# RichealYoung/BRIEF_PyTorch

Hardware: AMD Instinct MI355X
Metric: encode_voxels_per_sec (higher is better)
Workload: dtype f32; 1 GPU; SingleTask 512^3 synthetic uint16 volume, SIREN 4x256 (layers=5, features=256, w0=20), randompoint sample_size=100000, datal2, Adamax lr=1e-3; layers=5, features=256, sample_size=100000, params=198657

## Files before the change

__graft_entry__.py:

```python
import os
import subprocess
import sys

ROOT = os.path.dirname(os.path.abspath(__file__))
if ROOT not in sys.path:
    sys.path.insert(0, ROOT)


def build():
    from brief_pytorch_amd import _lib
    _lib.build(verbose=True)
    subprocess.check_call(["make", "-s", "-C", os.path.join(ROOT, "oracle")])
    import brief_pytorch_amd
    L = _lib.lib()
    for name in _lib.EXPORTS:
        assert hasattr(L, name), name
    print("build ok: libbrief_hip.so version", L.brief_version())


def smoke():
    import numpy as np
    import torch
    from brief_pytorch_amd import _lib
    from brief_pytorch_amd.networks import SIREN
    from brief_pytorch_amd.synthetic import make_volume
    from oracle import oracle as O

    assert torch.cuda.is_available(), "smoke() needs a GPU"
    _lib.lib()
    dims = (12, 16, 20)
    vol = make_volume(dims, seed=1)
    vn, side = O.normalize(vol)
    n = int(np.prod(dims))
    tv = torch.from_numpy(vn.reshape(-1, 1)).cuda()
    for layers, feats in ((5, 256), (4, 64), (3, 1100)):
        torch.manual_seed(0)
        m = SIREN(coords_channel=3, data_channel=1, features=feats, layers=layers, w0=20)
        d = O.make_desc(3, 1, layers, feats, 20.0)
        p = m.params.numpy().copy()
        m.to("cuda")
        loss, _ = m.train_step(n, tv, grid=(dims, -1.0, 1.0))
        lo, go, _, _ = O.loss_grad(d, p, O.grid_coords(dims), vn.reshape(-1, 1))
        g = m.grads.cpu().numpy()
        assert abs(loss.item() - lo) / lo < 1e-5, (loss.item(), lo)
# ... 12 lines not shown
```

brief_pytorch_amd/_lib.py:

```python
import ctypes as C
import os
import subprocess

_HERE = os.path.dirname(os.path.abspath(__file__))
LIB_PATH = os.environ.get("BRIEF_LIB", os.path.join(_HERE, "libbrief_hip.so"))
SRC = os.path.join(_HERE, "csrc", "brief_hip.hip")
_CSRC = os.path.join(_HERE, "csrc")
_DEPS = sorted(os.path.join(_CSRC, f) for f in (os.listdir(_CSRC) if os.path.isdir(_CSRC) else []) if f.endswith((".hip", ".inc", ".h"))) \
    + [os.path.join(os.path.dirname(_HERE), "include", "brief_hip.h")]
HIPCC = os.environ.get("HIPCC", "/opt/rocm/bin/hipcc")


class BriefError(RuntimeError):
    pass


class SirenDesc(C.Structure):
    _fields_ = [("cin", C.c_int32), ("cout", C.c_int32), ("layers", C.c_int32), ("features", C.c_int32),
                ("w0_first", C.c_float), ("w0_hidden", C.c_float), ("output_act", C.c_int32), ("precision", C.c_int32)]


class GridDesc(C.Structure):
    _fields_ = [("ndim", C.c_int32), ("reserved", C.c_int32), ("dims", C.c_int64 * 3), ("lo", C.c_float), ("hi", C.c_float)]

# ... 65 lines not shown

EXPORTS = ["brief_version", "brief_last_error", "brief_param_count", "brief_packed_count",
           "brief_train_workspace_bytes", "brief_siren_repack", "brief_siren_forward", "brief_forward_workspace_bytes", "brief_siren_forward_ws", "brief_siren_forward_box", "brief_siren_train_step", "brief_siren_fit_step",
           "brief_siren_fit", "brief_multi_fit",
           "brief_optim_step", "brief_sample_indices", "brief_sse_u16", "brief_profile_enable", "brief_profile_fused", "brief_deblock_edge", "brief_ssim_u16", "brief_ssim_partial_count",
           "brief_sincos_probe", "brief_cu_count",
           "brief_ffn_param_count", "brief_ffn_packed_count", "brief_ffn_train_workspace_bytes", "brief_ffn_repack", "brief_ffn_forward",
           "brief_ffn_forward_box", "brief_ffn_train_step", "brief_ffn_fit",
           "brief_nerf_param_count", "brief_nerf_packed_count", "brief_nerf_train_workspace_bytes", "brief_nerf_repack", "brief_nerf_forward",
           "brief_nerf_forward_box", "brief_nerf_train_step", "brief_nerf_fit",
           "brief_mfn_param_count", "brief_mfn_packed_count", "brief_mfn_train_workspace_bytes", "brief_mfn_repack", "brief_mfn_forward",
           "brief_mfn_forward_box", "brief_mfn_train_step", "brief_mfn_fit",
           "brief_taper_param_count", "brief_taper_packed_count", "brief_taper_train_workspace_bytes", "brief_taper_repack",
           "brief_taper_forward", "brief_taper_forward_box", "brief_taper_train_step", "brief_taper_fit",
           "brief_correct_chunk_elems", "brief_correct_count", "brief_correct_emit", "brief_correct_apply"]


def needs_build():
    if LIB_PATH != os.path.join(_HERE, "libbrief_hip.so"):
        return False
    if not os.path.exists(LIB_PATH):
        return True
    t = os.path.getmtime(LIB_PATH)
    return any(os.path.exists(d) and os.path.getmtime(d) > t for d in _DEPS)


DIAG_LIB_PATH = os.path.join(_HERE, "libbrief_hip_diag.so")


def build(force=False, verbose=False, diagnostics=False, defines=(), out=None):
    target = out or (DIAG_LIB_PATH if diagnostics else os.path.join(_HERE, "libbrief_hip.so"))
    if not force and not diagnostics and not defines and out is None and not needs_build():
        return LIB_PATH
    cmd = [HIPCC, "--offload-arch=gfx950", "-O3", "-std=c++17", "-ffp-contract=off", "-shared", "-fPIC", SRC, "-o", target]
    if diagnostics:
        cmd.append("-DBRIEF_DIAGNOSTICS")
    cmd += ["-D" + d for d in defines]
    if verbose:
        print(" ".join(cmd))
    subprocess.check_call(cmd)
    return target


_LIB = None


def lib():
    global _LIB
    if _LIB is not None:
        return _LIB
    import torch
    if not os.path.exists(LIB_PATH):
        raise BriefError("libbrief_hip.so is not built (run `python -c 'import __graft_entry__ as g; g.build()'`); "
                         "there is no CPU fallback for the fused SIREN path")
    L = C.CDLL(LIB_PATH)
    dp, gp, bp, vp = C.POINTER(SirenDesc), C.POINTER(GridDesc), C.POINTER(BatchDesc), C.c_void_p
    L.brief_version.restype = C.c_int
    if L.brief_version() != 130:
        raise BriefError("libbrief_hip.so is version %d, this binding needs 130 (brief_siren_forward_ws, widths to 4096): rebuild with __graft_entry__.build()" % L.brief_version())
    L.brief_last_error.restype = C.c_char_p
    L.brief_param_count.restype = C.c_int64
    L.brief_param_count.argtypes = [dp]
    L.brief_packed_count.restype = C.c_int64
    L.brief_packed_count.argtypes = [dp]
    L.brief_train_workspace_bytes.restype = C.c_int64
    L.brief_train_workspace_bytes.argtypes = [dp, C.c_int64]
# ... 89 lines not shown
```

brief_pytorch_amd/csrc/brief_device.inc:

```
typedef float f32x16 __attribute__((ext_vector_type(16)));
#define MFMA(a, b, c) __builtin_amdgcn_mfma_f32_32x32x2f32((a), (b), (c), 0, 0, 0)

#define ROWMAP(r, hi) (((r) & 3) + 8 * ((r) >> 2) + 4 * (hi))
template <int V> struct RoleC { static constexpr int value = V; };

template <int NT, bool INFER = false>
struct KCfg {
    static constexpr int WM = INFER ? brief_wm_infer(NT) : brief_wm(NT);
    static constexpr int WS = 4 / WM;
    static constexpr int MTW = (NT + WM - 1) / WM;
    static constexpr bool EXACT = (NT % WM) == 0;
    static constexpr int FP = 32 * NT;
    static constexpr int XS_FLOATS = WS * NT * 1024;
    static constexpr int TROWS = 32 * MTW;
    static constexpr int RS = (TROWS + 63) / 64;
    static constexpr int T_FLOATS = 4 * TROWS * 33;
    static constexpr int G_FLOATS = 4 * 256;
};

struct GridArgs {
    int ndim;
    int64_t dims[3];
    float lo, hi;
    float step[3];
// ... 12 lines not shown
    return dv == 1 ? nn : (uint32_t)__umul64hi(magic, (uint64_t)nn);
}

struct FusedArgs {
    brief_siren_desc d;
    const float *pk;
    const float *coords;
    const float *targets;
    const float *weights;
    const int64_t *idx;
    int64_t offset;
    int64_t n;
    uint64_t rng_pop, rng_seed, rng_step;
    GridArgs grid;
    int loss_kind;
    float thr, beta, inv_count;
    float *Z;
    float *D;
    int64_t npad;
    float *rec;
    int64_t n_begin, n_end;
    int rec_base;
    void *S16[5];
    float *slabs;
    float *yhat_out;
    void *out;
    int out_kind;
    float scale_min, den, span, vmin;
    int stagger_cus;
    int stagger;
    int pers_wgs;
    int64_t pers_tiles;
    int diag;
};
struct FusedBoxArgs : FusedArgs {
    BoxArgs box;
};
template <bool BOX> struct KArgsT { using type = FusedArgs; };
template <> struct KArgsT<true> { using type = FusedBoxArgs; };
typedef const __attribute__((address_space(4))) FusedBoxArgs *kargs_box;

__device__ __forceinline__ void lds_barrier()
{
    asm volatile("s_waitcnt lgkmcnt(0)" ::: "memory");
    __builtin_amdgcn_s_barrier();
    asm volatile("" ::: "memory");
}

__device__ __forceinline__ float lin_coord(const GridArgs &g, int a, int64_t i)
{
    const int64_t nn = g.dims[a];
    if (nn == 1) return g.lo;
    return i < nn / 2 ? __fmaf_rn(g.step[a], (float)i, g.lo) : __fmaf_rn(-g.step[a], (float)(nn - 1 - i), g.hi);
}

__device__ __forceinline__ float lin_coord32(const GridArgs &g, int a, uint32_t i)
{
    const uint32_t nn = (uint32_t)g.dims[a];
    if (nn == 1) return g.lo;
    return i < nn / 2 ? __fmaf_rn(g.step[a], (float)i, g.lo) : __fmaf_rn(-g.step[a], (float)(nn - 1 - i), g.hi);
}

__device__ __forceinline__ void grid_coords(const GridArgs &g, int cin, int64_t j, float &x0, float &x1, float &x2)
{
    if (cin == 3) {
        int64_t id, ih, iw;
        if (g.fast) {
// ... 135 lines not shown
                }
        }
        if (it + 1 < NIT) breg[it + 1] = Xs[(it + 1) * 64 + lane];
        __builtin_amdgcn_sched_barrier(0);
        const float4 b = breg[it];
#pragma unroll
        for (int t = 0; t < K::MTW; ++t) {
            if (K::EXACT || wm + K::WM * t < NT) {
                const float4 a = areg[it][t];
                acc[t] = MFMA(a.x, b.x, acc[t]);
                acc[t] = MFMA(a.y, b.y, acc[t]);
                acc[t] = MFMA(a.z, b.z, acc[t]);
                acc[t] = MFMA(a.w, b.w, acc[t]);
            }
        }
    }
}

template <int NT, bool INFER = false>
__device__ __forceinline__ void write_image(float4 *Xs, const f32x16 (&h)[(KCfg<NT, INFER>::MTW)], int wm, int lane)
{
    using K = KCfg<NT, INFER>;
#pragma unroll
    for (int t = 0; t < K::MTW; ++t) {
        const int mt = wm + K::WM * t;
        if (K::EXACT || mt < NT) {
#pragma unroll
            for (int q = 0; q < 4; ++q)
                Xs[(mt * 4 + q) * 64 + lane] = make_float4(h[t][4 * q], h[t][4 * q + 1], h[t][4 * q + 2], h[t][4 * q + 3]);
        }
    }
}

__device__ __forceinline__ void philox_round(uint32_t (&c)[4], uint32_t k0, uint32_t k1)
{
    const uint64_t p0 = (uint64_t)0xD2511F53u * c[0], p1 = (uint64_t)0xCD9E8D57u * c[2];
    const uint32_t n0 = (uint32_t)(p1 >> 32) ^ c[1] ^ k0, n1 = (uint32_t)p1;
    const uint32_t n2 = (uint32_t)(p0 >> 32) ^ c[3] ^ k1, n3 = (uint32_t)p0;
    c[0] = n0; c[1] = n1; c[2] = n2; c[3] = n3;
}

__device__ __forceinline__ int64_t philox_index(int64_t i, uint64_t pop, uint64_t seed, uint64_t step)
{
    uint32_t c[4] = {(uint32_t)i, (uint32_t)((uint64_t)i >> 32), (uint32_t)step, (uint32_t)(step >> 32)};
    uint32_t k0 = (uint32_t)seed, k1 = (uint32_t)(seed >> 32);
#pragma unroll
    for (int r = 0; r < 10; ++r) {
        philox_round(c, k0, k1);
        k0 += 0x9E3779B9u; k1 += 0xBB67AE85u;
    }
    const uint64_t r64 = ((uint64_t)c[0] << 32) | c[1];
    return (int64_t)__umul64hi(r64, pop);
}

#ifndef BRIEF_FUSED64
#ifndef BRIEF_LEAN_RM3
#define BRIEF_LEAN_RM3 1
#endif
#define BRIEF_FUSED64 0
#endif
#ifndef BRIEF_KERNARG_RELOAD
#define BRIEF_KERNARG_RELOAD 1
#endif
#ifndef BRIEF_TRAIN_WPE
#define BRIEF_TRAIN_WPE 2
#endif
// ... 6 lines not shown
```

brief_pytorch_amd/csrc/brief_fused.inc:

```
template <int NT, bool INFER = false>
struct FusedLds {
    using K = KCfg<NT, INFER>;
    static constexpr int R_FLOATS = K::XS_FLOATS > K::T_FLOATS ? K::XS_FLOATS : K::T_FLOATS;
    static constexpr int G_OFF = R_FLOATS;
    static constexpr int HW_OFF = G_OFF + K::G_FLOATS;
    static constexpr int TOTAL = HW_OFF + 4 * K::FP + 4;
};

#ifndef BRIEF_LEAN
#define BRIEF_LEAN 1
#endif
#ifndef BRIEF_LEAN7
#define BRIEF_LEAN7 0
#endif
constexpr bool fused_lean(int NT) { return BRIEF_LEAN && (NT == 8 || NT == BRIEF_LEAN7); }
constexpr int fused_train_wpe(int NT) { return NT > 8 ? 1 : (NT <= 4 || fused_lean(NT) ? (BRIEF_TRAIN_WPE > 3 ? BRIEF_TRAIN_WPE : 3) : BRIEF_TRAIN_WPE); }
template <int NT, bool TRAIN, bool BOX = false>
__global__ __launch_bounds__(256, TRAIN ? fused_train_wpe(NT) : (NT > 8 ? 2 : 3)) void k_fused(const typename KArgsT<BOX>::type a)
{
    static_assert(!(TRAIN && BOX), "the box mapping is an inference instantiation");
#ifdef BRIEF_STAMPS
    float st_acc[10] = {0.f, 0.f, 0.f, 0.f, 0.f, 0.f, 0.f, 0.f, 0.f, 0.f};
    long long st_last = clock64();
    const long long st_c0 = st_last, st_r0 = wall_clock64();
#endif
    using K = KCfg<NT, !TRAIN>;
    using LD = FusedLds<NT, !TRAIN>;
    extern __shared__ __attribute__((aligned(16))) float smem[];
    float4 *X = reinterpret_cast<float4 *>(smem);
    float *T = smem;
    float *G = smem + LD::G_OFF;
    float *HW = smem + LD::HW_OFF;

    const int lane = threadIdx.x & 63;
    const int wave = __builtin_amdgcn_readfirstlane(threadIdx.x >> 6);
    const int hi = lane >> 5, ln = lane & 31;
    const int wm = wave % K::WM, ws = wave / K::WM;
    const brief_siren_desc &d = a.d;
    const int L = d.layers, cin = d.cin, cout = d.cout;
    const int kit = (d.features + 7) >> 3;
    const int64_t npad = a.npad;
    const float *pk = a.pk;
    float4 *Xs = X + ws * (NT * 256);
    float *Tw = T + wave * (K::TROWS * 33);
    float *Gw = G + wave * 256;
    const float4 *W0p = reinterpret_cast<const float4 *>(pk + brief_pk_w0(d));
    const __amdgpu_buffer_rsrc_t rs_pk =
        __builtin_amdgcn_make_buffer_rsrc((void *)pk, 0, (int)(brief_pk_count(d) * 4), 0x00020000);
    const int stash_bytes = (a.diag & 1) ? 0 : (int)((int64_t)K::FP * npad * 4);
// ... 328 lines not shown
                if (K::EXACT || mt < NT) {
#pragma unroll
                    for (int r = 0; r < 16; ++r)
                        dl[t][r] = acc[t][r] * BRIEF_COS_REV(zr[t][r]);
                }
            }
        }
        STAMP(7)
        lds_barrier();
#pragma unroll
        for (int t = 0; t < K::MTW; ++t) {
#pragma unroll
            for (int r = 0; r < 16; ++r) Tw[(32 * t + ROWMAP(r, hi)) * 33 + ln] = dl[t][r];
        }
        lds_barrier();
#pragma unroll
        for (int rs = 0; rs < K::RS; ++rs) {
            float4 s0 = make_float4(0.f, 0.f, 0.f, 0.f);
            const int row = lane + 64 * rs;
            const float *trow = Tw + (row < K::TROWS ? row : 0) * 33;
#pragma unroll 4
            for (int s = 0; s < 32; ++s) {
                const float dv = trow[s];
                const float4 xv = *reinterpret_cast<const float4 *>(Gw + 128 + s * 4);
                s0.x = __fmaf_rn(dv, xv.x, s0.x); s0.y = __fmaf_rn(dv, xv.y, s0.y);
                s0.z = __fmaf_rn(dv, xv.z, s0.z); s0.w = __fmaf_rn(dv, xv.w, s0.w);
            }
            if (row < K::TROWS) { acc0[rs][0] += s0.x; acc0[rs][1] += s0.y; acc0[rs][2] += s0.z; acc0[rs][3] += s0.w; }
        }
        lds_barrier();
        STAMP(6)
    }
#undef FUSED_LOAD_BIAS
    if (TRAIN) {
        float *rec = a.rec + (((int64_t)blockIdx.x + a.rec_base) * 4 + wave) * BRIEF_REC_FLOATS;
#pragma unroll
        for (int rs = 0; rs < K::RS; ++rs) {
            const int row = lane + 64 * rs;
            if (row < 128) {
#pragma unroll
                for (int c = 0; c < 4; ++c) {
                    rec[row * 4 + c] = acc0[rs][c];
                    rec[BRIEF_REC_DWH + c * 128 + row] = accWh[rs][c];
                }
            }
        }
        for (int off = 32; off >= 1; off >>= 1) lsum += __shfl_xor(lsum, off);
        if (lane == 0) {
#pragma unroll
            for (int c = 0; c < 4; ++c) rec[BRIEF_REC_DBH + c] = accbh[c];
            rec[BRIEF_REC_LOSS] = lsum;
#ifdef BRIEF_STAMPS
            for (int i = 0; i < 10; ++i) rec[BRIEF_REC_STAMPS + i] = st_acc[i];
            rec[BRIEF_REC_STAMPS + 10] = (float)(clock64() - st_c0);
            rec[BRIEF_REC_STAMPS + 11] = (float)(wall_clock64() - st_r0);
            rec[BRIEF_REC_STAMPS + 12] = (float)(st_r0 & 0xFFFFFF);
            rec[BRIEF_REC_STAMPS + 13] = (float)(__builtin_amdgcn_s_getreg(20 | (0 << 6) | (3 << 11)) & 15);
            rec[BRIEF_REC_STAMPS + 14] = (float)(__builtin_amdgcn_s_getreg(4 | (0 << 6) | (15 << 11)) & 0xFFFF);
#endif
        }
    }
}
```

brief_pytorch_amd/csrc/brief_hip.hip:

```cpp
#include <hip/hip_runtime.h>
#include <hip/hip_ext.h>
#include <stdint.h>
#include <stdio.h>
#include <string.h>
#include <stdlib.h>
#include <mutex>
#include "brief_layout.h"
#include "brief_math.h"

#include "brief_device.inc"
#include "brief_fused.inc"
#include "brief_lean.inc"
#include "brief_wide.inc"
#include "brief_small.inc"
#include "brief_wgrad.inc"
#include "brief_x3.inc"
#include "brief_reduce.inc"
#include "brief_bf16.inc"
#include "brief_aux.inc"
#include "brief_ffn.inc"
#include "brief_nerf.inc"
#include "brief_mfn.inc"
#include "brief_taper.inc"
#include "brief_correct.inc"
// ... 117 lines not shown
static const bool g_wg_per_cu_set = env_str("BRIEF_WG_PER_CU") != nullptr;
static const int g_stagger = env_int("BRIEF_STAGGER", 0, 0, 64);
static const int g_diag = env_int("BRIEF_DIAG", 0, 0, 255);
static const int g_x3_decode = env_int("BRIEF_X3_DECODE", 1, 0, 1);
static const int g_wgrad_repeat = env_int("BRIEF_WGRAD_REPEAT", 1, 1, 8);
static const int g_reduce_sg_big = env_int("BRIEF_REDUCE_SG_BIG", 4, 1, 64);
static const int g_reduce_part = env_int("BRIEF_REDUCE_PART", 0, 0, 2);
static const int g_reduce_vec = env_int("BRIEF_REDUCE_VEC", 1, 0, 1);
static const int g_reduce_sg_small = env_int("BRIEF_REDUCE_SG", 0, 0, 64);
static int64_t fused_wg_samples(const brief_siren_desc &d, bool train)
{
    if (brief_use_wide(d)) return 32;
    if (d.precision == BRIEF_PREC_F32 && brief_use_lean(d, train)) return 32;
    if (!train && d.precision == BRIEF_PREC_F32) return 32 * (4 / brief_wm_infer(brief_nt(d)));
    return brief_wg_samples(brief_nt(d));
}
static int fused_grid(const brief_siren_desc &d, int64_t n, bool train)
{
    const int nt = brief_nt(d);
    const int64_t wgs_ = fused_wg_samples(d, train);
    const int64_t tiles = (n + wgs_ - 1) / wgs_;
    const int wpe = g_wg_per_cu_set ? g_wg_per_cu : (d.precision == BRIEF_PREC_BF16X3 && (train || g_x3_decode) ? 2  :
                    (BRIEF_FUSED64 && train && nt == 8 ? (BRIEF_FUSED64 == 1 ? 2 : 3)  : (train ? fused_train_wpe(nt) : (nt > 8 ? 2 : 3))));
    int64_t cap = (int64_t)kCUs * (train && nt > 8 ? 1 : wpe);
    if (brief_use_wide(d)) cap = kCUs;
    if (d.precision == BRIEF_PREC_F32 && brief_use_lean(d, train))
    {
        const int64_t by_lds = (160 * 1024) / (int64_t)(sizeof(float) * lean_lds(1, (nt + 3) / 4, nt).total);
        const int64_t by_regs = lean_wpe(1, (nt + 3) / 4);
        cap = (int64_t)kCUs * (by_lds < by_regs ? (by_lds > 0 ? by_lds : 1) : by_regs);
    }
    return (int)(tiles < cap ? (tiles > 0 ? tiles : 1) : cap);
}
struct FusedPlan { int grid, pers_wgs; int64_t pers_tiles; };
static const int g_tail_rounds = env_int("BRIEF_TAIL_ROUNDS", 0, 0, 64);
static FusedPlan fused_plan(const brief_siren_desc &d, int64_t n, bool train)
{
    const int nt = brief_nt(d);
    const int64_t wgs_ = fused_wg_samples(d, train);
    const int64_t tiles = (n + wgs_ - 1) / wgs_;
    const int cap = fused_grid(d, n, train);
    FusedPlan p;
    p.grid = cap; p.pers_wgs = cap; p.pers_tiles = tiles;
    if (!train || nt > 8 || tiles <= cap || brief_use_wide(d)) return p;
    if (g_tail_rounds == 0) return p;
    int64_t rounds = tiles / cap - g_tail_rounds;
    if (rounds < 0) rounds = 0;
    const int64_t max_wgs = (int64_t)kCUs * kRecWgsPerCu;
    while (tiles - rounds * cap + (rounds ? cap : 0) > max_wgs) ++rounds;
    if (rounds * cap >= tiles) return p;
    p.pers_wgs = rounds ? cap : 0;
    p.pers_tiles = rounds * cap;
    p.grid = p.pers_wgs + (int)(tiles - p.pers_tiles);
    return p;
}
#ifndef BRIEF_WGRAD_ROUNDS
#define BRIEF_WGRAD_ROUNDS 1
#endif
#ifndef BRIEF_TAIL_PLAN
#define BRIEF_TAIL_PLAN 1
#endif
#ifndef BRIEF_TAIL_LEAN
#define BRIEF_TAIL_LEAN 0
#endif
#ifndef BRIEF_TAIL_MODE_DEFAULT
#define BRIEF_TAIL_MODE_DEFAULT 2
#endif
#ifndef BRIEF_TAIL_R
#define BRIEF_TAIL_R 1.15
#define BRIEF_TAIL_R1 1.05
#endif
#ifndef BRIEF_TAIL_MIN_SPLITS
#define BRIEF_TAIL_MIN_SPLITS 6
#endif
#ifndef BRIEF_TAIL_MIN_ROUNDS
#define BRIEF_TAIL_MIN_ROUNDS 3
#endif
struct TailPlan { int mode ; bool on; int grid_body, grid_tail; int64_t tiles_body; int ns, n_norm; int64_t kfix_n, kfix_s; };
// ... 13 lines not shown
    const int64_t full = tiles / G * G, rem = tiles - full;
    if (full == 0 || rem == 0) return p;
    if (g_tail_mode == 2 && nt >= 9 && nt <= g_tail_ntmax && rem * 4 <= 3 * (int64_t)kCUs) {
        const int hidden = d.layers - 2, nq = wgrad_nq(nt), qt = (nt + nq - 1) / nq;
        const int64_t chunks = brief_npad_d(d, n) / 32, B = (int64_t)hidden * nq * nq;
        int ns = wgrad_split_rule(d, chunks, 1);
        if ((int64_t)ns * B > kCUs) ns = (int)(kCUs / B);
        const int per_xcd = kCUs / 8, tail_x = (int)((rem + 7) / 8);
        int n_norm = 0;
        if ((int64_t)ns * B <= kCUs)
            for (int c = ns - 1; c >= 1; --c) {
                const int a_ = (int)((c * B + 7) / 8), s_ = (int)(((ns - c) * B + 7) / 8);
                if (a_ + tail_x <= per_xcd && a_ + s_ <= per_xcd && (ns - c) * B >= rem) { n_norm = c; break; }
            }
        const int n_short = ns - n_norm;
        const double r = g_tail_r ? 0.01 * g_tail_r : (nt <= 16 ? BRIEF_TAIL_R : BRIEF_TAIL_R1);
        const double rho = r * 2.0 * hidden * nt * nt / (double)(qt * qt);
        const double k_norm = ((double)chunks + n_short * rho) / ns, k_short = k_norm - rho;
        if (n_norm > 0 && k_short >= 4.0 && rho < 0.8 * k_norm) {
            p.kfix_n = (int64_t)(k_norm * 65536.0); p.kfix_s = (int64_t)(k_short * 65536.0);
            const int64_t b_norm = ((int64_t)(ns - n_short) * p.kfix_n) >> 16;
            if (b_norm <= full && b_norm > 0) {
                p.mode = 2; p.on = true; p.grid_body = G; p.grid_tail = (int)rem; p.tiles_body = full; p.ns = ns; p.n_norm = ns - n_short;
                return p;
            }
        }
    }
    if (!(brief_use_wide(d) || (BRIEF_TAIL_LEAN && brief_use_lean(d, true) && nt >= 9))) return p;
    if (rem * 4 > 3 * (int64_t)G) return p;
    if (wgrad_split_rule(d, full, BRIEF_TAIL_MIN_ROUNDS) < BRIEF_TAIL_MIN_SPLITS) return p;
    p.mode = 1; p.on = true; p.grid_body = G; p.grid_tail = (int)rem; p.tiles_body = full;
    return p;
}
static int wgrad_split_rule(const brief_siren_desc &d, int64_t nchunks, int min_rounds)
{
    const int hidden = d.layers - 2;
    if (hidden <= 0) return 0;
    const int nq = wgrad_nq(brief_nt(d));
    const int64_t B = (int64_t)hidden * nq * nq;
    int64_t s = kWgradBlocks / B;
    if (s < 1) s = 1;
    if (min_rounds > 1) {
        double best = 1e30;
        for (int64_t c = 1; c <= 64; ++c) {
            const int64_t rounds = (c * B + kWgradBlocks - 1) / kWgradBlocks;
            if (rounds < min_rounds && c < 64) continue;
            const double cost = (double)rounds / (double)c + 0.0001 * (double)c;
            if (cost < best - 1e-9) { best = cost; s = c; }
        }
    } else if (brief_nt(d) > 32) {
        double best = 1e30;
        for (int64_t c = 1; c <= 16; ++c) {
            const double cost = (double)((c * B + kWgradBlocks - 1) / kWgradBlocks) / (double)c + 0.001 * (double)c;
            if (cost < best - 1e-9) { best = cost; s = c; }
        }
    } else if (nq >= 2 && BRIEF_WGRAD_ROUNDS) {
        const double base = 1.0 / (double)s + 0.0001 * (double)s;
        double best = base;
        const int64_t cmax = 4 * s > 16 ? 4 * s : 16;
        for (int64_t c = s + 1; c <= cmax && c <= 64; ++c) {
            const double cost = (double)((c * B + kWgradBlocks - 1) / kWgradBlocks) / (double)c + 0.0001 * (double)c;
            if (cost < best - 1e-9 && cost < 0.985 * base) { best = cost; s = c; }
        }
    }
    if (s > nchunks) s = nchunks;
    return (int)s;
// ... 587 lines not shown
            hipLaunchKernelGGL(k_reduce, dim3(nbh), dim3(256), 0, st, ra, nbh);
            HIP_TRY(hipGetLastError());
        }
        Reduce16Args r16;
        memset(&r16, 0, sizeof(r16));
        r16.d = *d; r16.slabs = ws + w16.slabs + (int64_t)hidden * nsp * (FP * FP + FP); r16.nsplit = nsp_s;
        r16.rec = fa.rec; r16.nwg = g16; r16.grads = grads; r16.loss_out = loss_out; r16.inv_count = inv16;
        if (upd) { r16.update = 1; r16.opt = upd->opt; r16.params = upd->params; r16.s1 = upd->s1; r16.s2 = upd->s2; r16.pk = upd->pk; }
        const int64_t items = l0c + (int64_t)d->cout * d->features + d->cout + 1;
        hipLaunchKernelGGL(k_reduce16, dim3((unsigned)((items + 3) / 4)), dim3(256), 0, st, r16);
        HIP_TRY(hipGetLastError());
        return 0;
    }
    const bool small = use_small(*d);
    const FusedPlan fp = fused_plan(*d, batch->n, true);
    TailPlan tp;
    memset(&tp, 0, sizeof(tp));
    if (!small) tp = fused_tail_plan(*d, batch->n);
    const int grid1 = small ? small_grid(*d, batch->n) : (tp.on ? tp.grid_body + tp.grid_tail : fp.grid);
    const int nsplit = small ? (d->layers > 2 ? grid1 : 0) : wgrad_splits(*d, batch->n);
    const float inv_count = (float)(1.0 / ((double)batch->n * d->cout));

    FusedArgs fa;
    memset(&fa, 0, sizeof(fa));
    fa.d = *d; fa.pk = packed;
    fa.coords = batch->coords; fa.targets = batch->targets; fa.weights = batch->weights;
    fa.idx = batch->idx; fa.offset = batch->offset; fa.n = batch->n;
    if (!batch->idx && batch->rng_pop > 0) { fa.rng_pop = (uint64_t)batch->rng_pop; fa.rng_seed = batch->rng_seed; fa.rng_step = batch->rng_step; }
    fill_grid(fa.grid, grid);
    fa.loss_kind = loss_kind; fa.thr = thr; fa.beta = beta; fa.inv_count = inv_count;
    fa.Z = ws + wl.z; fa.D = ws + wl.dd; fa.npad = brief_npad_d(*d, batch->n);
    fa.rec = ws + wl.rec; fa.slabs = brief_use_wide(*d) ? ws + wl.img : ws + wl.slabs; fa.yhat_out = yhat_out;
    fa.stagger_cus = kCUs; fa.stagger = g_stagger; fa.diag = g_diag;
    fa.pers_wgs = fp.pers_wgs; fa.pers_tiles = fp.pers_tiles;
    ReduceArgs ra;
    memset(&ra, 0, sizeof(ra));
    ra.d = *d; ra.rec = fa.rec; ra.nrec_wg = grid1; ra.slabs = ws + wl.slabs; ra.nsplit = nsplit;
    int sg_small = 8;
    while (sg_small < 32 && sg_small * 16 < nsplit) sg_small *= 2;
    if (g_reduce_sg_small > 0) sg_small = g_reduce_sg_small;
    ra.sgroups = small ? sg_small : g_reduce_sg_big;
    const int rthreads = 256;
    ra.grads = grads; ra.loss_out = loss_out; ra.inv_count = inv_count;
    if (upd) { ra.update = 1; ra.opt = upd->opt; ra.params = upd->params; ra.s1 = upd->s1; ra.s2 = upd->s2; ra.pk = upd->pk; }
    const int64_t l0_count = (int64_t)d->features * d->cin + d->features;
    const int64_t hcount = brief_canon_head_off(*d) - l0_count;
    const int64_t skinny = d->features + (int64_t)d->cout * ((d->features + 3) / 4) + 2;
    ra.vec = (!small && g_reduce_vec && d->precision == BRIEF_PREC_F32 && rthreads * 4 <= 1024) ? (d->features % 4 == 0 ? 4 : (d->features % 2 == 0 ? 2 : 0)) : 0;
    {
        const uintptr_t bits = (uintptr_t)grads | (uintptr_t)ra.params | (uintptr_t)ra.s1 | (uintptr_t)ra.s2 | (uintptr_t)ra.pk | (uintptr_t)ra.slabs;
        while (ra.vec > 1 && bits % (sizeof(float) * ra.vec) != 0) ra.vec /= 2;
        if (ra.vec == 1) ra.vec = 0;
    }
    const int ppb = rthreads / ra.sgroups * (ra.vec ? ra.vec : 1);
    const int nb_hidden = (int)((hcount + ppb - 1) / ppb);
    const int wpb = rthreads / 64;
    const int nb_skinny = (int)((skinny + wpb - 1) / wpb);
    if (plan_only) {
        if (!small) return fail(BRIEF_ERR_INVALID, "internal: step plans exist for narrow nets only");
        plan_only->fa = fa; plan_only->ra = ra; plan_only->grid1 = grid1; plan_only->nb_hidden = nb_hidden;
        plan_only->nb_reduce = nb_hidden + nb_skinny; plan_only->nt = nt; plan_only->hb = small_hb(*d);
        return 0;
    }
    const bool prof = prof_live();
    hipEvent_t pe0 = prof ? dev_state()->prof_ev[2 * g_prof_n] : nullptr, pe1 = prof ? dev_state()->prof_ev[2 * g_prof_n + 1] : nullptr;
    if (small) {
        const int hb = small_hb(*d);
// ... 1650 lines not shown
```

Measured before the change: 101.9 million voxels/s.

## Process leftover samples as 16-wide half tiles with 16x16x4 MFMA

For the persistent fused training kernel (NT=8, lean path), the partial last round of 32-sample tiles is now handled as 16-sample half tiles, spread over up to one per CU. These use a new 16x16x4 MFMA chain for the forward and backward passes, with stash and weight-gradient accumulation adapted to match. The goal is to cut the wasted work and load imbalance of a mostly empty final round. It adds a sizeable duplicate code path with its own indexing and pad handling, which raises the risk of correctness bugs. The build also compiles the diagnostics library in parallel and skips rebuilding it when it is up to date.

```diff
diff --git a/__graft_entry__.py b/__graft_entry__.py
--- a/__graft_entry__.py
+++ b/__graft_entry__.py
@@ -8,8 +8,12 @@
 
 
 def build():
+    from concurrent.futures import ThreadPoolExecutor
     from brief_pytorch_amd import _lib
-    _lib.build(verbose=True)
+    with ThreadPoolExecutor(1) as pool:
+        diag = pool.submit(_lib.build, verbose=True, diagnostics=True)
+        _lib.build(verbose=True)
+        diag.result()
     subprocess.check_call(["make", "-s", "-C", os.path.join(ROOT, "oracle")])
     import brief_pytorch_amd
     L = _lib.lib()
diff --git a/brief_pytorch_amd/_lib.py b/brief_pytorch_amd/_lib.py
--- a/brief_pytorch_amd/_lib.py
+++ b/brief_pytorch_amd/_lib.py
@@ -121,6 +121,9 @@
     target = out or (DIAG_LIB_PATH if diagnostics else os.path.join(_HERE, "libbrief_hip.so"))
     if not force and not diagnostics and not defines and out is None and not needs_build():
         return LIB_PATH
+    if not force and diagnostics and not defines and out is None and os.path.exists(target) \
+            and all(os.path.getmtime(d) <= os.path.getmtime(target) for d in _DEPS if os.path.exists(d)):
+        return target
     cmd = [HIPCC, "--offload-arch=gfx950", "-O3", "-std=c++17", "-ffp-contract=off", "-shared", "-fPIC", SRC, "-o", target]
     if diagnostics:
         cmd.append("-DBRIEF_DIAGNOSTICS")
diff --git a/brief_pytorch_amd/csrc/brief_device.inc b/brief_pytorch_amd/csrc/brief_device.inc
--- a/brief_pytorch_amd/csrc/brief_device.inc
+++ b/brief_pytorch_amd/csrc/brief_device.inc
@@ -68,7 +68,9 @@
     int pers_wgs;
     int64_t pers_tiles;
     int diag;
-};
+    int half_n;
+};
+static_assert(offsetof(FusedArgs, half_n) + sizeof(int) == sizeof(FusedArgs), "half_n sits in the tail padding behind diag");
 struct FusedBoxArgs : FusedArgs {
     BoxArgs box;
 };
@@ -270,6 +272,59 @@
     }
 }
 
+typedef float f32x4 __attribute__((ext_vector_type(4)));
+#define MFMAH(a, b, c) __builtin_amdgcn_mfma_f32_16x16x4f32((a), (b), (c), 0, 0, 0)
+
+template <int NT>
+__device__ __forceinline__ void chain_half(f32x4 (&acc)[(KCfg<NT>::MTW)][2], __amdgpu_buffer_rsrc_t rs, int soff_layer ,
+                                           const float4 *Xs, int wm, int lane, int kit)
+{
+    using K = KCfg<NT>;
+    constexpr int NIT = NT * 4;
+    constexpr int PD = NIT < 8 ? NIT : 8;
+    const int i = lane & 15, kk = lane >> 4;
+    const int voff = ((kk & 1) * 32 + i) * 16 + (kk >> 1) * 4;
+    const float *Xf = reinterpret_cast<const float *>(Xs) + ((kk & 1) * 32 + i) * 4 + (kk >> 1);
+    int soff_w = soff_layer + wm * (NT * 4 * 1024);
+    asm volatile("" : "+s"(soff_w));
+    float areg[NIT][K::MTW][2][2];
+    float breg[NIT][2];
+#define CHAIN_HALF_LOAD(it_)                                                                                       \
+    _Pragma("unroll") for (int t = 0; t < K::MTW; ++t)                                                             \
+        _Pragma("unroll") for (int hf = 0; hf < 2; ++hf)                                                           \
+            _Pragma("unroll") for (int u = 0; u < 2; ++u)                                                          \
+                areg[it_][t][hf][u] = bload1(rs, voff + 256 * hf + 8 * u, soff_w + (K::WM * t * NT * 4 + (it_)) * 1024);
+#pragma unroll
+    for (int it = 0; it < PD; ++it) CHAIN_HALF_LOAD(it)
+    breg[0][0] = Xf[0]; breg[0][1] = Xf[2];
+#pragma unroll
+    for (int it = 0; it < NIT; ++it) {
+        if (it >= NIT - 3 && it >= kit) break;
+        if (it + PD < NIT) CHAIN_HALF_LOAD(it + PD)
+        if (it + 1 < NIT) { breg[it + 1][0] = Xf[(it + 1) * 256]; breg[it + 1][1] = Xf[(it + 1) * 256 + 2]; }
+        __builtin_amdgcn_sched_barrier(0);
+#pragma unroll
+        for (int u = 0; u < 2; ++u)
+#pragma unroll
+            for (int t = 0; t < K::MTW; ++t)
+#pragma unroll
+                for (int hf = 0; hf < 2; ++hf) acc[t][hf] = MFMAH(areg[it][t][hf][u], breg[it][u], acc[t][hf]);
+    }
+#undef CHAIN_HALF_LOAD
+}
+
+template <int NT>
+__device__ __forceinline__ void write_image_half(float4 *Xs, const f32x4 (&h)[(KCfg<NT>::MTW)][2], int wm, int lane)
+{
+    using K = KCfg<NT>;
+    const int col = lane & 15, g = lane >> 4;
+#pragma unroll
+    for (int t = 0; t < K::MTW; ++t)
+#pragma unroll
+        for (int hf = 0; hf < 2; ++hf)
+            Xs[((wm + K::WM * t) * 4 + 2 * hf + (g >> 1)) * 64 + 32 * (g & 1) + col] = make_float4(h[t][hf][0], h[t][hf][1], h[t][hf][2], h[t][hf][3]);
+}
+
 __device__ __forceinline__ void philox_round(uint32_t (&c)[4], uint32_t k0, uint32_t k1)
 {
     const uint64_t p0 = (uint64_t)0xD2511F53u * c[0], p1 = (uint64_t)0xCD9E8D57u * c[2];
diff --git a/brief_pytorch_amd/csrc/brief_fused.inc b/brief_pytorch_amd/csrc/brief_fused.inc
--- a/brief_pytorch_amd/csrc/brief_fused.inc
+++ b/brief_pytorch_amd/csrc/brief_fused.inc
@@ -13,8 +13,272 @@
 #ifndef BRIEF_LEAN7
 #define BRIEF_LEAN7 0
 #endif
+#ifndef BRIEF_HALF_TILE
+#define BRIEF_HALF_TILE 1
+#endif
 constexpr bool fused_lean(int NT) { return BRIEF_LEAN && (NT == 8 || NT == BRIEF_LEAN7); }
 constexpr int fused_train_wpe(int NT) { return NT > 8 ? 1 : (NT <= 4 || fused_lean(NT) ? (BRIEF_TRAIN_WPE > 3 ? BRIEF_TRAIN_WPE : 3) : BRIEF_TRAIN_WPE); }
+template <int NT>
+__device__ __forceinline__ void fused_half_tile(float (&acc0)[(KCfg<NT>::RS)][4], float (&accWh)[(KCfg<NT>::RS)][4], float (&accbh)[4], float &lsum)
+{
+    using K = KCfg<NT>;
+    using LD = FusedLds<NT>;
+    static_assert(K::EXACT && K::RS == 1 && K::WS == 1, "the half-tile walk is written for whole feature tiles, 64 features per wave");
+    extern __shared__ __attribute__((aligned(16))) float smem[];
+    int tid = threadIdx.x;
+    asm volatile("" : "+v"(tid));
+    const int lane = tid & 63;
+    const int wm = __builtin_amdgcn_readfirstlane(tid >> 6);
+    float4 *Xs = reinterpret_cast<float4 *>(smem);
+    float *Tw = smem + wm * (K::TROWS * 33);
+    float *Gw = smem + LD::G_OFF + wm * 256;
+    const float *HW = smem + LD::HW_OFF;
+    typedef const __attribute__((address_space(4))) FusedArgs *kargs_f;
+    kargs_f ap = (kargs_f)__builtin_amdgcn_kernarg_segment_ptr();
+    asm volatile("" : "+s"(ap));
+    brief_siren_desc d;
+    d.cin = ap->d.cin; d.cout = ap->d.cout; d.layers = ap->d.layers; d.features = ap->d.features;
+    d.w0_first = ap->d.w0_first; d.w0_hidden = ap->d.w0_hidden; d.output_act = ap->d.output_act; d.precision = ap->d.precision;
+    const int L = d.layers, cin = d.cin, cout = d.cout;
+    const int kit = (d.features + 7) >> 3;
+    const float *pk = ap->pk;
+    const __amdgpu_buffer_rsrc_t rs_pk =
+        __builtin_amdgcn_make_buffer_rsrc((void *)pk, 0, (int)(brief_pk_count(d) * 4), 0x00020000);
+    const int64_t npad = ap->npad;
+    const int stash_bytes = (ap->diag & 1) ? 0 : (int)((int64_t)K::FP * npad * 4);
+    const int col = lane & 15, g4 = lane >> 4, hi = g4 & 1;
+    const int hb = (int)blockIdx.x;
+    const int64_t s0 = ap->pers_tiles * 32 + 16 * (int64_t)hb;
+    const int64_t n = s0 + col;
+    const bool valid = n < ap->n;
+    const int voff_s = (int)((s0 >> 5) * (K::FP * 128)) + (((int)s0 & 16) + col) * 4 + g4 * 4 * 128;
+    const bool pad_mate = hb == ap->half_n - 1 && !(hb & 1);
+#define HALF_STASH_STORE(v, rsrc)                                                                       \
+    _Pragma("unroll") for (int t = 0; t < K::MTW; ++t)                                                  \
+        _Pragma("unroll") for (int hf = 0; hf < 2; ++hf)                                                \
+            _Pragma("unroll") for (int r = 0; r < 4; ++r) {                                             \
+                bstore1(v[t][hf][r], rsrc, voff_s, (32 * (wm + K::WM * t) + 16 * hf + r) * 128);        \
+                if (pad_mate) bstore1(0.f, rsrc, voff_s + 64, (32 * (wm + K::WM * t) + 16 * hf + r) * 128); \
+            }
+    int64_t j = 0;
+    if (valid) j = ap->idx ? ap->idx[n] : (ap->rng_pop ? philox_index(n, ap->rng_pop, ap->rng_seed, ap->rng_step) : n + ap->offset);
+    float x0 = 0.f, x1 = 0.f, x2 = 0.f;
+    float yv[4] = {0.f, 0.f, 0.f, 0.f}, wv4[4] = {1.f, 1.f, 1.f, 1.f};
+    if (valid) {
+        const float *k_tg = ap->targets, *k_wt = ap->weights, *k_co = ap->coords;
+#pragma unroll
+        for (int c = 0; c < 4; ++c) {
+            if (c < cout) {
+                yv[c] = k_tg[j * cout + c];
+                if (k_wt) wv4[c] = k_wt[j * cout + c];
+            }
+        }
+        if (k_co) {
+            x0 = k_co[j * cin];
+            x1 = k_co[j * cin + 1];
+            if (cin == 3) x2 = k_co[j * cin + 2];
+        } else {
+            GridArgs kg;
+            kg.ndim = ap->grid.ndim; kg.lo = ap->grid.lo; kg.hi = ap->grid.hi; kg.fast = ap->grid.fast;
+#pragma unroll
+            for (int ax = 0; ax < 3; ++ax) { kg.dims[ax] = ap->grid.dims[ax]; kg.step[ax] = ap->grid.step[ax]; kg.magic[ax] = ap->grid.magic[ax]; }
+            grid_coords(kg, cin, j, x0, x1, x2);
+        }
+    }
+    f32x4 acc[K::MTW][2], hreg[K::MTW][2], creg[K::MTW][2];
+    {
+        const float bx = g4 == 0 ? x0 : (g4 == 1 ? x1 : (g4 == 2 ? x2 : 1.0f));
+        const float *W0f = pk + brief_pk_w0(d);
+#pragma unroll
+        for (int t = 0; t < K::MTW; ++t)
+#pragma unroll
+            for (int hf = 0; hf < 2; ++hf) {
+#pragma unroll
+                for (int r = 0; r < 4; ++r) { acc[t][hf][r] = 0.f; hreg[t][hf][r] = 0.f; creg[t][hf][r] = 0.f; }
+                acc[t][hf] = MFMAH(W0f[(32 * (wm + K::WM * t) + 16 * hf + col) * 4 + g4], bx, acc[t][hf]);
+            }
+    }
+    for (int l = 0; l <= L - 2; ++l) {
+        const bool last = (l == L - 2);
+        if (l > 0) {
+            const float *bp_ = pk + brief_pk_hidden(d, l) + 2 * K::FP * K::FP;
+#pragma unroll
+            for (int t = 0; t < K::MTW; ++t)
+#pragma unroll
+                for (int hf = 0; hf < 2; ++hf) {
+                    const float4 b = *reinterpret_cast<const float4 *>(bp_ + 32 * (wm + K::WM * t) + 16 * hf + 4 * g4);
+                    acc[t][hf][0] = b.x; acc[t][hf][1] = b.y; acc[t][hf][2] = b.z; acc[t][hf][3] = b.w;
+                }
+            __builtin_amdgcn_s_setprio(3);
+            chain_half<NT>(acc, rs_pk, (int)(brief_pk_hidden(d, l) * 4), Xs, wm, lane, kit);
+            __builtin_amdgcn_s_setprio(0);
+            lds_barrier();
+        }
+#pragma unroll
+        for (int t = 0; t < K::MTW; ++t)
+#pragma unroll
+            for (int hf = 0; hf < 2; ++hf)
+#pragma unroll
+                for (int r = 0; r < 4; ++r) acc[t][hf][r] = __builtin_amdgcn_fractf(acc[t][hf][r]);
+        if (!last) {
+            const __amdgpu_buffer_rsrc_t rz =
+                __builtin_amdgcn_make_buffer_rsrc((void *)(ap->Z + (int64_t)l * K::FP * npad), 0, stash_bytes, 0x00020000);
+            HALF_STASH_STORE(acc, rz)
+        }
+#pragma unroll
+        for (int t = 0; t < K::MTW; ++t)
+#pragma unroll
+            for (int hf = 0; hf < 2; ++hf)
+#pragma unroll
+                for (int r = 0; r < 4; ++r) {
+                    hreg[t][hf][r] = BRIEF_SIN_REV(acc[t][hf][r]);
+                    if (last) creg[t][hf][r] = BRIEF_COS_REV(acc[t][hf][r]);
+                }
+        write_image_half<NT>(Xs, hreg, wm, lane);
+        lds_barrier();
+    }
+    float zo[4], yh[4], g[4];
+#pragma unroll
+    for (int c = 0; c < 4; ++c) {
+        zo[c] = 0.f; yh[c] = 0.f; g[c] = 0.f;
+        if (c < cout) {
+            float p = 0.f;
+            const float *wrow = HW + c * K::FP;
+#pragma unroll
+            for (int kt = 0; kt < NT; ++kt) {
+#pragma unroll
+                for (int q = 0; q < 4; ++q) {
+                    const float4 hv = Xs[(kt * 4 + q) * 64 + 32 * hi + col];
+                    const float4 wv = *reinterpret_cast<const float4 *>(wrow + 32 * kt + 8 * q + 4 * hi);
+                    p = __fmaf_rn(wv.x, hv.x, p); p = __fmaf_rn(wv.y, hv.y, p);
+                    p = __fmaf_rn(wv.z, hv.z, p); p = __fmaf_rn(wv.w, hv.w, p);
+                }
+            }
+            p += __shfl_xor(p, 16);
+            zo[c] = p + HW[4 * K::FP + c];
+            yh[c] = d.output_act ? brief_fast_sinf(d.w0_hidden * zo[c]) : zo[c];
+        }
+    }
+    {
+        const int loss_kind = ap->loss_kind;
+        const float thr = ap->thr, beta = ap->beta, inv_count = ap->inv_count;
+        float *yhat_out = ap->yhat_out;
+#pragma unroll
+        for (int c = 0; c < 4; ++c) {
+            if (c < cout && valid) {
+                float we = wv4[c];
+                if (thr != 0.f && yh[c] <= thr) we = 1.0f;
+                const float df = yh[c] - yv[c];
+                float li, gi;
+                if (loss_kind == BRIEF_LOSS_L2) { li = df * df; gi = 2.0f * df; }
+                else if (loss_kind == BRIEF_LOSS_SMOOTHL1) {
+                    const float ad = fabsf(df);
+                    if (ad < beta) { li = 0.5f * df * df / beta; gi = df / beta; }
+                    else { li = ad - 0.5f * beta; gi = df < 0.f ? -1.0f : 1.0f; }
+                } else { li = 0.f; gi = 0.f; }
+                if (wm == 0 && g4 == 0) lsum += li * we;
+                g[c] = loss_kind == BRIEF_LOSS_EXTERNAL ? yv[c] : gi * we * inv_count;
+                if (d.output_act) g[c] *= d.w0_hidden * brief_fast_cosf(d.w0_hidden * zo[c]);
+                if (yhat_out && wm == 0 && g4 == 0) yhat_out[n * cout + c] = yh[c];
+            }
+        }
+    }
+    lds_barrier();
+#pragma unroll
+    for (int t = 0; t < K::MTW; ++t)
+#pragma unroll
+        for (int hf = 0; hf < 2; ++hf)
+#pragma unroll
+            for (int r = 0; r < 4; ++r) Tw[(32 * t + 16 * hf + 4 * g4 + r) * 33 + col] = hreg[t][hf][r];
+    if (g4 == 0) *reinterpret_cast<float4 *>(Gw + col * 4) = make_float4(g[0], g[1], g[2], g[3]);
+    else if (g4 == 1) *reinterpret_cast<float4 *>(Gw + 128 + col * 4) = make_float4(x0, x1, x2, 1.0f);
+    lds_barrier();
+    {
+        float4 sW = make_float4(0.f, 0.f, 0.f, 0.f), sb = make_float4(0.f, 0.f, 0.f, 0.f);
+        const float *trow = Tw + lane * 33;
+#pragma unroll 4
+        for (int s = 0; s < 16; ++s) {
+            const float hv = trow[s];
+            const float4 gv = *reinterpret_cast<const float4 *>(Gw + s * 4);
+            sW.x = __fmaf_rn(hv, gv.x, sW.x); sW.y = __fmaf_rn(hv, gv.y, sW.y);
+            sW.z = __fmaf_rn(hv, gv.z, sW.z); sW.w = __fmaf_rn(hv, gv.w, sW.w);
+            sb.x += gv.x; sb.y += gv.y; sb.z += gv.z; sb.w += gv.w;
+        }
+        accWh[0][0] += sW.x; accWh[0][1] += sW.y; accWh[0][2] += sW.z; accWh[0][3] += sW.w;
+        accbh[0] += sb.x; accbh[1] += sb.y; accbh[2] += sb.z; accbh[3] += sb.w;
+    }
+    f32x4 dl[K::MTW][2];
+    {
+        const float om_top = (L - 2) == 0 ? d.w0_first : d.w0_hidden;
+        float gom[4];
+#pragma unroll
+        for (int c = 0; c < 4; ++c) gom[c] = om_top * g[c];
+#pragma unroll
+        for (int t = 0; t < K::MTW; ++t)
+#pragma unroll
+            for (int hf = 0; hf < 2; ++hf) {
+                float4 sacc = make_float4(0.f, 0.f, 0.f, 0.f);
+#pragma unroll
+                for (int c = 0; c < 4; ++c) {
+                    if (c < cout) {
+                        const float4 wv = *reinterpret_cast<const float4 *>(HW + c * K::FP + 32 * (wm + K::WM * t) + 16 * hf + 4 * g4);
+                        sacc.x = __fmaf_rn(wv.x, gom[c], sacc.x); sacc.y = __fmaf_rn(wv.y, gom[c], sacc.y);
+                        sacc.z = __fmaf_rn(wv.z, gom[c], sacc.z); sacc.w = __fmaf_rn(wv.w, gom[c], sacc.w);
+                    }
+                }
+                dl[t][hf][0] = creg[t][hf][0] * sacc.x; dl[t][hf][1] = creg[t][hf][1] * sacc.y;
+                dl[t][hf][2] = creg[t][hf][2] * sacc.z; dl[t][hf][3] = creg[t][hf][3] * sacc.w;
+            }
+    }
+    for (int l = L - 2; l >= 1; --l) {
+        const __amdgpu_buffer_rsrc_t rd =
+            __builtin_amdgcn_make_buffer_rsrc((void *)(ap->D + (int64_t)(l - 1) * K::FP * npad), 0, stash_bytes, 0x00020000);
+        HALF_STASH_STORE(dl, rd)
+        const __amdgpu_buffer_rsrc_t rzp =
+            __builtin_amdgcn_make_buffer_rsrc((void *)(ap->Z + (int64_t)(l - 1) * K::FP * npad), 0, stash_bytes, 0x00020000);
+        lds_barrier();
+        write_image_half<NT>(Xs, dl, wm, lane);
+        lds_barrier();
+#pragma unroll
+        for (int t = 0; t < K::MTW; ++t)
+#pragma unroll
+            for (int hf = 0; hf < 2; ++hf)
+#pragma unroll
+                for (int r = 0; r < 4; ++r) acc[t][hf][r] = 0.f;
+        __builtin_amdgcn_s_setprio(3);
+        chain_half<NT>(acc, rs_pk, (int)((brief_pk_hidden(d, l) + K::FP * K::FP) * 4), Xs, wm, lane, kit);
+        __builtin_amdgcn_s_setprio(0);
+#pragma unroll
+        for (int t = 0; t < K::MTW; ++t)
+#pragma unroll
+            for (int hf = 0; hf < 2; ++hf)
+#pragma unroll
+                for (int r = 0; r < 4; ++r)
+                    dl[t][hf][r] = acc[t][hf][r] * BRIEF_COS_REV(bload1s(rzp, voff_s, (32 * (wm + K::WM * t) + 16 * hf + r) * 128));
+    }
+#undef HALF_STASH_STORE
+    lds_barrier();
+#pragma unroll
+    for (int t = 0; t < K::MTW; ++t)
+#pragma unroll
+        for (int hf = 0; hf < 2; ++hf)
+#pragma unroll
+            for (int r = 0; r < 4; ++r) Tw[(32 * t + 16 * hf + 4 * g4 + r) * 33 + col] = dl[t][hf][r];
+    lds_barrier();
+    {
+        float4 s0 = make_float4(0.f, 0.f, 0.f, 0.f);
+        const float *trow = Tw + lane * 33;
+#pragma unroll 4
+        for (int s = 0; s < 16; ++s) {
+            const float dv = trow[s];
+            const float4 xv = *reinterpret_cast<const float4 *>(Gw + 128 + s * 4);
+            s0.x = __fmaf_rn(dv, xv.x, s0.x); s0.y = __fmaf_rn(dv, xv.y, s0.y);
+            s0.z = __fmaf_rn(dv, xv.z, s0.z); s0.w = __fmaf_rn(dv, xv.w, s0.w);
+        }
+        acc0[0][0] += s0.x; acc0[0][1] += s0.y; acc0[0][2] += s0.z; acc0[0][3] += s0.w;
+    }
+}
+
 template <int NT, bool TRAIN, bool BOX = false>
 __global__ __launch_bounds__(256, TRAIN ? fused_train_wpe(NT) : (NT > 8 ? 2 : 3)) void k_fused(const typename KArgsT<BOX>::type a)
 {
@@ -409,6 +673,12 @@
         STAMP(6)
     }
 #undef FUSED_LOAD_BIAS
+    if constexpr (BRIEF_HALF_TILE && TRAIN && NT == 8 && fused_lean(NT)) {
+        typedef const __attribute__((address_space(4))) FusedArgs *kargs_h;
+        kargs_h hp = (kargs_h)__builtin_amdgcn_kernarg_segment_ptr();
+        asm volatile("" : "+s"(hp));
+        if ((int)blockIdx.x < hp->half_n) fused_half_tile<NT>(acc0, accWh, accbh, lsum);
+    }
     if (TRAIN) {
         float *rec = a.rec + (((int64_t)blockIdx.x + a.rec_base) * 4 + wave) * BRIEF_REC_FLOATS;
 #pragma unroll
diff --git a/brief_pytorch_amd/csrc/brief_hip.hip b/brief_pytorch_amd/csrc/brief_hip.hip
--- a/brief_pytorch_amd/csrc/brief_hip.hip
+++ b/brief_pytorch_amd/csrc/brief_hip.hip
@@ -173,8 +173,10 @@
     }
     return (int)(tiles < cap ? (tiles > 0 ? tiles : 1) : cap);
 }
-struct FusedPlan { int grid, pers_wgs; int64_t pers_tiles; };
+struct FusedPlan { int grid, pers_wgs; int64_t pers_tiles; int half_n; };
 static const int g_tail_rounds = env_int("BRIEF_TAIL_ROUNDS", 0, 0, 64);
+static const int g_half_tiles = env_int("BRIEF_HALF_TILES", 1, 0, 1);
+static bool fused_tail_on(const brief_siren_desc &d, int64_t n);
 static FusedPlan fused_plan(const brief_siren_desc &d, int64_t n, bool train)
 {
     const int nt = brief_nt(d);
@@ -182,9 +184,15 @@
     const int64_t tiles = (n + wgs_ - 1) / wgs_;
     const int cap = fused_grid(d, n, train);
     FusedPlan p;
-    p.grid = cap; p.pers_wgs = cap; p.pers_tiles = tiles;
+    p.grid = cap; p.pers_wgs = cap; p.pers_tiles = tiles; p.half_n = 0;
     if (!train || nt > 8 || tiles <= cap || brief_use_wide(d)) return p;
-    if (g_tail_rounds == 0) return p;
+    if (g_tail_rounds == 0) {
+        if (BRIEF_HALF_TILE && g_half_tiles && nt == 8 && fused_lean(8) && !BRIEF_FUSED64 && d.precision == BRIEF_PREC_F32 && !fused_tail_on(d, n)) {
+            const int64_t r = tiles / cap, rem = n - r * cap * 32, H = (rem + 15) / 16;
+            if (H > 0 && H <= kCUs) { p.pers_tiles = r * cap; p.half_n = (int)H; }
+        }
+        return p;
+    }
     int64_t rounds = tiles / cap - g_tail_rounds;
     if (rounds < 0) rounds = 0;
     const int64_t max_wgs = (int64_t)kCUs * kRecWgsPerCu;
@@ -264,6 +272,7 @@
     p.mode = 1; p.on = true; p.grid_body = G; p.grid_tail = (int)rem; p.tiles_body = full;
     return p;
 }
+static bool fused_tail_on(const brief_siren_desc &d, int64_t n) { return fused_tail_plan(d, n).on; }
 static int wgrad_split_rule(const brief_siren_desc &d, int64_t nchunks, int min_rounds)
 {
     const int hidden = d.layers - 2;
@@ -917,7 +926,7 @@
     fa.Z = ws + wl.z; fa.D = ws + wl.dd; fa.npad = brief_npad_d(*d, batch->n);
     fa.rec = ws + wl.rec; fa.slabs = brief_use_wide(*d) ? ws + wl.img : ws + wl.slabs; fa.yhat_out = yhat_out;
     fa.stagger_cus = kCUs; fa.stagger = g_stagger; fa.diag = g_diag;
-    fa.pers_wgs = fp.pers_wgs; fa.pers_tiles = fp.pers_tiles;
+    fa.pers_wgs = fp.pers_wgs; fa.pers_tiles = fp.pers_tiles; fa.half_n = tp.on ? 0 : fp.half_n;
     ReduceArgs ra;
     memset(&ra, 0, sizeof(ra));
     ra.d = *d; ra.rec = fa.rec; ra.nrec_wg = grid1; ra.slabs = ws + wl.slabs; ra.nsplit = nsplit;
```

After: 98.58 million voxels/s. -3.3%, worse.
